# tsinghua-fib-lab/DRL-urban-planning

Measured on NVIDIA H100. Metric: ppo_update_graph_samples_per_sec, higher is better.
Workload: dtype f32

## Files before the change

drl_urban_planning_b200/csrc/optim_kernels.cuh:

```cuda
#pragma once
#include <cuda_runtime.h>
#include <stdint.h>

#include "../../include/upb200.h"
#include "layout.h"

namespace upb {

template <class L>
__device__ __forceinline__ bool chain_owns(int col) {
  return (col >= L::chain0_begin && col < L::chain0_end) || (col >= L::chain1_begin && col < L::chain1_end);
}

template <class L>
__device__ __forceinline__ bool write_grad_col(float* grad, int col, float v) {
  bool param = false;
  if (col < L::num_params && !chain_owns<L>(col)) { grad[col] = v; param = true; }
  else if (col >= L::num_params && col < L::stat_offset) grad[col] = 0.f;
  if (col >= L::stats && col < L::stats + UPB_STAT_COUNT)
    grad[L::stat_offset + (col - L::stats)] = stat_summed(col - L::stats) ? v : 0.f;
  return param;
}

constexpr int KL_STOP_SLOT = 13;
// ... 40 lines not shown
}

__device__ __forceinline__ double gclip_block_tree(double s, double* red) {
#pragma unroll
  for (int o = 16; o > 0; o >>= 1) s += __shfl_xor_sync(0xffffffffu, s, o);
  if ((threadIdx.x & 31) == 0) red[threadIdx.x >> 5] = s;
  __syncthreads();
  double r = 0.0;
  if (threadIdx.x == 0)
    for (int w = 0; w < GCLIP_BLOCK / 32; ++w) r += red[w];
  return r;
}

__device__ __forceinline__ float gclip_norm(const double* parts, int n) {
  double s = 0.0;
  for (int i = 0; i < n; ++i) s += parts[i];
  return (float)sqrt(s);
}

__device__ __forceinline__ float gclip_coef(float norm, float max_norm) {
  const float c = __fmul_rn(__frcp_rn(__fadd_rn(norm, 1e-6f)), max_norm);
  return c > 1.f ? 1.f : c;
}

template <class L>
__device__ __forceinline__ float column_sum4(const float* __restrict__ gpart, int nparts, int col) {
  float s0 = 0.f, s1 = 0.f, s2 = 0.f, s3 = 0.f;
  int c = 0;
  for (; c + 4 <= nparts; c += 4) {
    s0 += gpart[(size_t)(c + 0) * L::row + col];
    s1 += gpart[(size_t)(c + 1) * L::row + col];
    s2 += gpart[(size_t)(c + 2) * L::row + col];
    s3 += gpart[(size_t)(c + 3) * L::row + col];
  }
  for (; c < nparts; ++c) s0 += gpart[(size_t)c * L::row + col];
  return (s0 + s1) + (s2 + s3);
}

__device__ __forceinline__ void attention_chain(int t, const float* sG, const float* sWin, const float* sW,
                                                const float* sB, float* gW, int w_stride, float* gWin, float* gB,
                                                int b_stride, float* gBin) {
  const int r = t >> 4, c = t & 15;
  const int gC[3] = {0, 272, 528};
  const int gBo[3] = {256, -1, 784};
#pragma unroll
  for (int s = 0; s < 3; ++s) {
    const float* Win = sWin + s * 256;
    const float* gc = sG + gC[s];
    const float* W = sW + s * 256;
    float a = 0.f, b = 0.f;
#pragma unroll
    for (int rr = 0; rr < 16; ++rr) {
      a = fmaf(Win[rr * 16 + r], gc[rr * 16 + c], a);
      b = fmaf(gc[r * 16 + rr], W[c * 16 + rr], b);
    }
    if (gBo[s] >= 0) b = fmaf(sG[gBo[s] + r], sB[s * 16 + c], b);
    gW[s * w_stride + t] = a;
    gWin[s * 256 + t] = b;
    if (t < 16) {
      float gb = 0.f, gbin = 0.f;
      if (gBo[s] >= 0) {
        for (int rr = 0; rr < 16; ++rr) gb = fmaf(Win[rr * 16 + t], sG[gBo[s] + rr], gb);
        gbin = sG[gBo[s] + t];
      }
      gB[s * b_stride + t] = gb;
      gBin[s * 16 + t] = gbin;
    }
  }
}

constexpr int RF_THREADS = 256;
constexpr int RF_BLOCKS = (G_ROW + RF_THREADS - 1) / RF_THREADS;
static_assert(P_ATT_K_W - P_ATT_Q_W == P_ATT_V_W - P_ATT_K_W && P_ATT_K_B - P_ATT_Q_B == P_ATT_V_B - P_ATT_K_B,
              "q / k / v projections at a fixed stride");

__global__ void __launch_bounds__(RF_THREADS) k_reduce_finish(const float* __restrict__ gpart, int nparts,
                                                              float* __restrict__ gsum, const float* __restrict__ P,
                                                              float* __restrict__ grad, unsigned int* ticket,
                                                              const unsigned int* kl_stop) {
  __shared__ float sG[816];
  __shared__ float sWin[768];
  __shared__ float sW[768];
  __shared__ float sB[48];
  __shared__ bool is_last;
  const int t = threadIdx.x;
  const int idx = blockIdx.x * RF_THREADS + t;
  if (kl_stop && kl_stop_set(kl_stop)) {
    if (idx < UPB_GRAD_STRIDE) write_skip_elem(grad, UPB_STAT_OFFSET, idx);
    return;
  }
  if (idx < G_ROW) {
    const float v = column_sum4<SgnnRow>(gpart, nparts, idx);
    gsum[idx] = v;
    write_grad_col<SgnnRow>(grad, idx, v);
  }
  __threadfence();
  __syncthreads();
  if (t == 0) is_last = (atomicAdd(ticket, 1u) == gridDim.x - 1);
  __syncthreads();
  if (!is_last) return;
  __threadfence();
  if (t == 0) *ticket = 0u;
  for (int i = t; i < 816; i += RF_THREADS) sG[i] = __ldcg(gsum + G_QC + i);
  for (int i = t; i < 768; i += RF_THREADS) sWin[i] = P[P_MHA_IN_W + i];
  sW[t] = P[P_ATT_Q_W + t];
  sW[256 + t] = P[P_ATT_K_W + t];
  sW[512 + t] = P[P_ATT_V_W + t];
  if (t < 16) { sB[t] = P[P_ATT_Q_B + t]; sB[16 + t] = P[P_ATT_K_B + t]; sB[32 + t] = P[P_ATT_V_B + t]; }
  __syncthreads();
  attention_chain(t, sG, sWin, sW, sB, grad + P_ATT_Q_W, P_ATT_K_W - P_ATT_Q_W, grad + P_MHA_IN_W, grad + P_ATT_Q_B,
                  P_ATT_K_B - P_ATT_Q_B, grad + P_MHA_IN_B);
}

struct ApplyArgs {
  float* params;
  float* grad;
  float* m;
  float* v;
  const long long* steps_in;
  long long* steps_out;
  float lr, beta1, beta2, eps;
  float weight_decay;
  int clip_now;
  int num_params, encoder_end, policy_end, lu_begin, rd_begin, stat_offset;
  unsigned int* kl_stop;
  float kl_limit;
  float max_norm;
  int nslice;
  int chain0_begin, chain0_end, chain1_begin, chain1_end;
  int nonfinite_guard;
};

constexpr int AP_THREADS = 512;
constexpr int AP_PER_THREAD = 2;
constexpr int AP_BLOCKS = (NUM_PARAMS + AP_THREADS * AP_PER_THREAD - 1) / (AP_THREADS * AP_PER_THREAD);

__device__ __forceinline__ float block_sum_ap(float v, float* red) {
#pragma unroll
  for (int o = 16; o > 0; o >>= 1) v += __shfl_xor_sync(0xffffffffu, v, o);
  if ((threadIdx.x & 31) == 0) red[threadIdx.x >> 5] = v;
  __syncthreads();
  float s = 0.f;
  for (int w = 0; w < AP_THREADS / 32; ++w) s += red[w];
  __syncthreads();
  return s;
}

static_assert(AP_THREADS == GCLIP_BLOCK, "k_apply forms the chain partial with the chain CTA's tree");
constexpr int GCLIP_MAX_PARTS = 128;
__device__ __noinline__ float apply_gclip_norm(const ApplyArgs& a) {
  __shared__ double parts[GCLIP_MAX_PARTS];
  __shared__ double red[GCLIP_BLOCK / 32];
  __shared__ float norm;
  const int t = threadIdx.x, lane = t & 31;
  for (int sl = t >> 5; sl < a.nslice; sl += AP_THREADS / 32) {
    double x[4];
#pragma unroll
    for (int k = 0; k < 4; ++k) {
      const int col = sl * SLICE + lane + 32 * k;
      const bool real = col < a.num_params && !(col >= a.chain0_begin && col < a.chain0_end) &&
// ... 217 lines not shown
```

drl_urban_planning_b200/csrc/sgnn_kernel.cuh:

```cuda
#pragma once
#include <cuda_runtime.h>
#include <math_constants.h>
#include <stdint.h>

#include "blob.h"
#include "layout.h"
#include "optim_kernels.cuh"

namespace upb {

constexpr int NT = 512;
constexpr int NW = NT / 32;
constexpr int NS = 464;
constexpr int AS = 5632;
constexpr int KS = 160;
constexpr int CH = 96;
constexpr float MASK_FILL = -4294967296.0f;
constexpr float EPS_DEG = 1e-6f;

constexpr int S_WET = 0;
constexpr int S_BE = S_WET + 384;
constexpr int S_WPQ0 = S_BE + 16;
constexpr int S_B0 = S_WPQ0 + 512;
constexpr int S_WPQ1 = S_B0 + 16;
// ... 120 lines not shown
struct StepArgs {
  const uint8_t* blob;
  const int* ids;
  int count;
  const float* params;
  const float* actions;
  const float* adv;
  const float* ret;
  const float* fixed_lp;
  const float* exps;
  float inv_batch, inv_ind;
  float clip_lo, clip_hi;
  float c_value, c_entropy;
  int diagnostics;
  float* out_value;
  float* out_logp;
  float* out_entropy;
  int* out_greedy;
  const float* uniforms;
  int* out_sample;
  float* gpart;
  float* scratch;
  size_t scratch_stride;
  int n_cap, e_cap;
  int fuse_tail;
  float* params_rw;
  float* grad_out;
  float* adam_m;
  float* adam_v;
  const long long* steps_in;
  long long* steps_out;
  unsigned int* gridbar;
  unsigned int bar_target;
  float lr, beta1, beta2, adam_eps;
  float weight_decay;
  int world, rank;
  unsigned int seq;
  float* const* peers;
  long long* stamps;
  const int* logit_rows;
  float* lu_logits;
  float* rd_logits;
  unsigned int* kl_stop;
  float kl_limit;
  const float* old_values;
  float value_clip;
  float max_norm;
  float* out_cand_logp;
  const float* old_cand_logp;
  float kl_coef;
  int nonfinite_guard;
};

__device__ __forceinline__ float ex2_approx(float x) {
  float y;
  asm("ex2.approx.ftz.f32 %0, %1;" : "=f"(y) : "f"(x));
  return y;
}
__device__ __forceinline__ float rcp_approx(float x) {
  float y;
  asm("rcp.approx.ftz.f32 %0, %1;" : "=f"(y) : "f"(x));
  return y;
}
__device__ __forceinline__ float exp2a(float a) {
  const float t = fminf(fmaxf(a * 2.8853900817779268f, -115.41560327111707f), 115.41560327111707f);
  return ex2_approx(t);
}
__device__ __forceinline__ void cp_async16(void* smem_dst, const void* gsrc) {
  const unsigned d = (unsigned)__cvta_generic_to_shared(smem_dst);
  asm volatile("cp.async.cg.shared.global [%0], [%1], 16;" ::"r"(d), "l"(gsrc) : "memory");
}
__device__ __forceinline__ void cp_async_commit() { asm volatile("cp.async.commit_group;" ::: "memory"); }
__device__ __forceinline__ void cp_async_wait_all() { asm volatile("cp.async.wait_group 0;" ::: "memory"); }

__device__ __forceinline__ unsigned smem_u32(const void* p) { return (unsigned)__cvta_generic_to_shared(p); }
__device__ __forceinline__ void mbar_init(uint64_t* bar, unsigned count) {
  asm volatile("mbarrier.init.shared::cta.b64 [%0], %1;" ::"r"(smem_u32(bar)), "r"(count) : "memory");
}
__device__ __forceinline__ void fence_mbar_init() { asm volatile("fence.mbarrier_init.release.cluster;" ::: "memory"); }
__device__ __forceinline__ void fence_proxy_async() { asm volatile("fence.proxy.async;" ::: "memory"); }
__device__ __forceinline__ void mbar_expect_tx(uint64_t* bar, unsigned bytes) {
  asm volatile("mbarrier.arrive.expect_tx.shared::cta.b64 _, [%0], %1;" ::"r"(smem_u32(bar)), "r"(bytes) : "memory");
}
__device__ __forceinline__ void bulk_g2s(void* smem_dst, const void* gsrc, unsigned bytes, uint64_t* bar) {
  asm volatile("cp.async.bulk.shared::cluster.global.mbarrier::complete_tx::bytes [%0], [%1], %2, [%3];"
               ::"r"(smem_u32(smem_dst)), "l"(gsrc), "r"(bytes), "r"(smem_u32(bar)) : "memory");
}
__device__ __forceinline__ void mbar_wait(uint64_t* bar, unsigned parity) {
  asm volatile(
      "{\n\t.reg .pred p;\n\t"
      "WAIT_%=:\n\t"
      "mbarrier.try_wait.parity.shared::cta.b64 p, [%0], %1;\n\t"
      "@p bra DONE_%=;\n\t"
      "bra WAIT_%=;\n\t"
      "DONE_%=:\n\t}"
      ::"r"(smem_u32(bar)), "r"(parity) : "memory");
}

__device__ __forceinline__ float4 ld4(const float* p) { return *reinterpret_cast<const float4*>(p); }
__device__ __forceinline__ void st4(float* p, float4 v) { *reinterpret_cast<float4*>(p) = v; }
__device__ __forceinline__ float4 f4(float a) { return make_float4(a, a, a, a); }
__device__ __forceinline__ float4 operator+(float4 a, float4 b) { return make_float4(a.x + b.x, a.y + b.y, a.z + b.z, a.w + b.w); }
__device__ __forceinline__ float4 operator*(float4 a, float s) { return make_float4(a.x * s, a.y * s, a.z * s, a.w * s); }
__device__ __forceinline__ float4 operator*(float4 a, float4 b) { return make_float4(a.x * b.x, a.y * b.y, a.z * b.z, a.w * b.w); }
__device__ __forceinline__ float dot4(float4 a, float4 b) { return a.x * b.x + a.y * b.y + a.z * b.z + a.w * b.w; }
__device__ __forceinline__ float comp(const float4& v, int j) { return j == 0 ? v.x : j == 1 ? v.y : j == 2 ? v.z : v.w; }
// ... 1770 lines not shown
      } else if (sh.stop && col == L::stats + KL_STOP_SLOT) {
        a.grad_out[L::stat_offset + KL_STOP_SLOT] = 1.f;
        *a.kl_stop = 1u;
      }
    }
    __syncthreads();
  }
}

__device__ __forceinline__ void tail_write_steps(const StepArgs& a, const TailShared& sh) {
  const int tid = threadIdx.x;
  const bool live_lu = sh.bits & 1u, live_rd = sh.bits & 2u;
  if (sh.timeout == 0 && !sh.stop)
    a.steps_out[tid] = tid == 0 ? a.steps_in[0] + 1
                                : sh.steps[(tid - 1) * 2 + (tid == 1 ? 1 : (tid == 2 ? (live_lu ? 1 : 0) : (live_rd ? 1 : 0)))];
  else
    a.steps_out[tid] = a.steps_in[tid];
}

__device__ __forceinline__ void tail_count_timeout(const StepArgs& a, const TailShared& sh) {
  if (threadIdx.x == 0 && sh.timeout) atomicAdd(a.gridbar + 6, 1u);
}

template <class L>
__device__ __noinline__ void tail_kl_gate(const StepArgs& a, TailShared& sh, const float* pull, const unsigned* myflags,
                                          bool sys) {
  if ((int)threadIdx.x < a.world) tail_poll(a, sh, myflags, threadIdx.x, L::stats / SLICE, sys);
  __syncthreads();
  if (threadIdx.x == 0) {
    float s4 = ld_relaxed(pull + L::stats + 4, sys), s8 = ld_relaxed(pull + L::stats + 8, sys);
    for (int p = 1; p < a.world; ++p) {
      s4 += ld_relaxed(pull + (size_t)p * G_ROW + L::stats + 4, sys);
      s8 += ld_relaxed(pull + (size_t)p * G_ROW + L::stats + 8, sys);
    }
    sh.stop = sh.timeout == 0 && kl_exceeds(s8, s4, a.kl_limit);
  }
  __syncthreads();
}

template <bool STEPS>
__device__ __forceinline__ void tail_chain_grads(const StepArgs& a, TailShared& sh, const float* pull,
                                                 const unsigned* myflags, bool sys, float* chain) {
  float* sG = chain;
  float* sWin = sG + 816;
  float* sW3 = sWin + 768;
  float* sB = sW3 + 768;
  float* sOut = sB + 48;
  const int tid = threadIdx.x, world = a.world;
  {
    constexpr int NCH = CHAIN_S1 - CHAIN_S0 + 1;
    if (tid < world * NCH) tail_poll(a, sh, myflags, tid % world, CHAIN_S0 + tid / world, sys);
    __syncthreads();
  }
  if constexpr (STEPS) {
    if (tid < 4) tail_write_steps(a, sh);
  }
  {
    float v0[MAX_PEERS], v1[MAX_PEERS];
#pragma unroll
    for (int p = 0; p < MAX_PEERS; ++p) {
      v0[p] = 0.f; v1[p] = 0.f;
      if (p < world) {
        v0[p] = ld_relaxed(pull + (size_t)p * G_ROW + G_QC + tid, sys);
        if (tid + NT < 816) v1[p] = ld_relaxed(pull + (size_t)p * G_ROW + G_QC + tid + NT, sys);
      }
    }
    float s0 = v0[0], s1 = v1[0];
#pragma unroll
    for (int p = 1; p < MAX_PEERS; ++p) if (p < world) { s0 += v0[p]; s1 += v1[p]; }
    sG[tid] = s0;
    if (tid + NT < 816) sG[tid + NT] = s1;
  }
  __syncthreads();
  if (tid < 256) attention_chain(tid, sG, sWin, sW3, sB, sOut, 256, sOut + 768, sOut + 1536, 16, sOut + 1584);
  __syncthreads();
}

template <class L>
__device__ __forceinline__ void tail_gclip(const StepArgs& a, TailShared& sh, const float* pull,
                                           const unsigned* myflags, bool sys, int c, bool active, double* sq,
                                           float* chain) {
  constexpr bool CHAIN = L::chain0_end > L::chain0_begin;
  constexpr int NPARTS = L::nslice + (CHAIN ? 1 : 0);
  static_assert(NPARTS <= FLAG_STRIDE, "a flag word per partial");
  double* const sparts = sq + SLICE;
  float& snorm = *reinterpret_cast<float*>(sparts + FLAG_STRIDE);
  float& scoef = *(&snorm + 1);
  const int tid = threadIdx.x, world = a.world;
  const unsigned par = a.seq & 1u;
  float* const mine = a.peers[a.rank];
  double* const parts = reinterpret_cast<double*>(mine + XCHG_GCLIP) + (size_t)par * FLAG_STRIDE;
  unsigned* const pflags = reinterpret_cast<unsigned*>(mine + XCHG_GCLIP_FLAGS) + (size_t)par * FLAG_STRIDE;
  const bool stop = sh.stop;

  for (int sl = blockIdx.x; sl < L::nslice; sl += gridDim.x) {
    if (tid < world) tail_poll(a, sh, myflags, tid, sl, sys);
    __syncthreads();
    const int col = sl * SLICE + c;
    if (active) {
      double x = 0.0;
      if (L::row % SLICE == 0 || col < L::row) {
        const float s = rank_sum(pull, world, col, sys);
        if (write_grad_col<L>(a.grad_out, col, s)) x = (double)s * (double)s;
        else if (stop && col == L::stats + KL_STOP_SLOT) {
          a.grad_out[L::stat_offset + KL_STOP_SLOT] = 1.f;
          *a.kl_stop = 1u;
// ... 58 lines not shown
  __syncthreads();

  const float norm = snorm, coef = scoef;
  const bool bad = a.nonfinite_guard && !isfinite(norm);
  const bool dead = sh.timeout != 0 || bad;
  const bool live_lu = sh.bits & 1u, live_rd = sh.bits & 2u;
  if (active) {
    for (int sl = blockIdx.x; sl < L::nslice; sl += gridDim.x) {
      const int col = sl * SLICE + c;
      if (col < L::num_params && !chain_owns<L>(col)) {
        int seg = 0;
        bool live = true;
        if (col >= L::lu_begin && col < L::rd_begin) { seg = 1; live = live_lu; }
        else if (col >= L::rd_begin && col < L::policy_end) { seg = 2; live = live_rd; }
        if (live && !dead)
          adam_elem(a, col, __fmul_rn(a.grad_out[col], coef), a.adam_m[col], a.adam_v[col], a.params_rw[col],
                    sh.adam[(seg * 2 + 1) * 2], sh.adam[(seg * 2 + 1) * 2 + 1]);
      } else if (col == L::stats + GCLIP_NORM_SLOT && !dead && a.max_norm > 0.f) {
        a.grad_out[L::stat_offset + GCLIP_NORM_SLOT] = norm;
      } else if (col == L::stats + NONFINITE_SLOT && bad && sh.timeout == 0) {
        a.grad_out[L::stat_offset + NONFINITE_SLOT] = 1.f;
      }
    }
  }
  if constexpr (CHAIN) {
    if (chain != nullptr && !dead) {
      const float* sOut = chain + 2400;
#pragma unroll
      for (int j = 0; j < 4; ++j) {
        const int i = tid + j * GCLIP_BLOCK;
        if (i < CHAIN_ELEMS) {
          const int dst = chain_dst(i);
          adam_elem(a, dst, __fmul_rn(sOut[i], coef), a.adam_m[dst], a.adam_v[dst], a.params_rw[dst], sh.adam[2],
                    sh.adam[3]);
        }
      }
    }
  }
}

template <class L>
__device__ __noinline__ void skip_step(const StepArgs& a) {
  if (!a.fuse_tail) return;
  const int tid = threadIdx.x;
  for (int i = blockIdx.x * blockDim.x + tid; i < L::stat_offset + UPB_STAT_COUNT; i += gridDim.x * blockDim.x)
    write_skip_elem(a.grad_out, L::stat_offset, i);
  if (blockIdx.x == 0) {
    if (tid < 4) a.steps_out[tid] = a.steps_in[tid];
    if (tid == 4) a.gridbar[2 + ((a.seq & 1u) ^ 1u)] = 0u;
  }
  grid_arrive(a.gridbar);
}

template <bool GCLIP>
__device__ __forceinline__ void fused_tail(const StepArgs& a, float* smem, unsigned stage_bits) {
  const int tid = threadIdx.x;
  const int nparts = gridDim.x;
  const int world = a.world, me = a.rank;
  const bool sys = world > 1;
  const unsigned par = a.seq & 1u;
  const bool chain_cta = blockIdx.x == gridDim.x - 1;
  __shared__ TailShared sh;
#define UPB_TSTAMP(ID) do { if (a.stamps != nullptr && blockIdx.x == 0 && threadIdx.x == 0) a.stamps[ID] = clock64(); } while (0)
  UPB_TSTAMP(40);
  float* const mine = a.peers[me];
  const float* const pull = mine + (size_t)par * MAX_PEERS * G_ROW;
  const unsigned* const myflags = reinterpret_cast<const unsigned*>(mine + XCHG_FLAGS) + (size_t)par * MAX_PEERS * FLAG_STRIDE;
  tail_prologue(a, sh, stage_bits);
  const int col0 = blockIdx.x * SLICE + (tid >> 2), part = tid & 3;
  float pm = 0.f, pv = 0.f, pp = 0.f;
  if (!GCLIP && part == 0 && col0 < NUM_PARAMS && !chain_owns<SgnnRow>(col0)) {
    pm = a.adam_m[col0]; pv = a.adam_v[col0]; pp = a.params_rw[col0];
  }
  float* sG = smem;
  float* sWin = sG + 816;
  float* sW3 = sWin + 768;
  float* sB = sW3 + 768;
  float* sOut = sB + 48;
  const int pW[3] = {P_ATT_Q_W, P_ATT_K_W, P_ATT_V_W};
  const int pB[3] = {P_ATT_Q_B, P_ATT_K_B, P_ATT_V_B};
  float cm[4], cv[4], cp[4];
  int cdst[4];
  if (chain_cta) {
    const float* P = a.params_rw;
    for (int i = tid; i < 768; i += NT) sWin[i] = P[P_MHA_IN_W + i];
    if (tid < 256) { sW3[tid] = P[P_ATT_Q_W + tid]; sW3[256 + tid] = P[P_ATT_K_W + tid]; sW3[512 + tid] = P[P_ATT_V_W + tid]; }
    if (tid < 16) { sB[tid] = P[P_ATT_Q_B + tid]; sB[16 + tid] = P[P_ATT_K_B + tid]; sB[32 + tid] = P[P_ATT_V_B + tid]; }
#pragma unroll
    for (int j = 0; j < 4; ++j) {
      const int i = tid + j * NT;
      int dst = 0;
      if (i < 768) dst = pW[i >> 8] + (i & 255);
      else if (i < 1536) dst = P_MHA_IN_W + (i - 768);
      else if (i < 1584) dst = pB[(i - 1536) >> 4] + ((i - 1536) & 15);
      else if (i < 1632) dst = P_MHA_IN_B + (i - 1584);
      cdst[j] = dst;
      if (!GCLIP && i < 1632) { cm[j] = a.adam_m[dst]; cv[j] = a.adam_v[dst]; cp[j] = P[dst]; }
    }
  }
  const unsigned flagword = tail_barrier(a);
  UPB_TSTAMP(41);

  float* sPart = smem + 4096;
  for (int sl = blockIdx.x; sl < NSLICE; sl += gridDim.x) {
    const int lane = tid & 31, warp = tid >> 5, cg = warp & 3, rg = warp >> 2;
    const float* src = a.gpart + sl * SLICE + cg * 32 + lane;
    float s = 0.f;
    for (int r0 = rg; r0 < nparts; r0 += 160) {
      float t[40];
#pragma unroll
      for (int j = 0; j < 40; ++j) t[j] = r0 + 4 * j < nparts ? __ldcg(src + (size_t)(r0 + 4 * j) * G_ROW) : 0.f;
#pragma unroll
      for (int w = 1; w < 40; w <<= 1)
#pragma unroll
        for (int j = 0; j + w < 40; j += 2 * w) t[j] += t[j + w];
      s += t[0];
    }
    __syncthreads();
    sPart[rg * SLICE + cg * 32 + lane] = s;
    __syncthreads();
    if (tid < SLICE) {
      const float v = (sPart[tid] + sPart[SLICE + tid]) + (sPart[2 * SLICE + tid] + sPart[3 * SLICE + tid]);
      const int col = sl * SLICE + tid;
      for (int r = 0; r < world; ++r) st_relaxed(sh.push[r] + col, v, sys);
    }
  }
  tail_release<SgnnRow>(a, flagword, NT, sys);
  if (a.kl_stop) tail_kl_gate<SgnnRow>(a, sh, pull, myflags, sys);
  UPB_TSTAMP(42);
  if constexpr (GCLIP) {
    tail_gclip<SgnnRow>(a, sh, pull, myflags, sys, tid >> 2, part == 0, reinterpret_cast<double*>(sPart + 4 * SLICE),
                        chain_cta ? smem : nullptr);
    if (chain_cta && tid < 4) tail_write_steps(a, sh);
    tail_count_timeout(a, sh);
    return;
  }

  tail_reduce_adam<SgnnRow>(a, sh, pull, myflags, sys, tid >> 2, part == 0, col0, pm, pv, pp);
  UPB_TSTAMP(43);
  if (!chain_cta) {
    tail_count_timeout(a, sh);
    return;
  }

  tail_chain_grads<true>(a, sh, pull, myflags, sys, sG);
  const bool dead = sh.timeout != 0 || sh.stop;
#pragma unroll
  for (int j = 0; j < 4; ++j) {
    const int i = tid + j * NT;
    if (i < 1632) {
      const float g = sOut[i];
      a.grad_out[cdst[j]] = g;
      if (!dead) adam_elem(a, cdst[j], g, cm[j], cv[j], cp[j], sh.adam[2], sh.adam[3]);
    }
  }
  tail_count_timeout(a, sh);
  UPB_TSTAMP(44);
}

template <bool TRAIN, bool GCLIP>
__device__ __forceinline__ void sgnn_step(const StepArgs& a) {
  extern __shared__ __align__(16) float smem[];
  __shared__ __align__(8) uint64_t s_mbar[4];
  if constexpr (TRAIN) {
    if (a.kl_stop && kl_stop_set(a.kl_stop)) {
      skip_step<SgnnRow>(a);
      return;
    }
  }
  const long long t_cta0 = a.stamps ? clock64() : 0;
  if (a.stamps && threadIdx.x == 0 && blockIdx.x == 0) {
    unsigned long long gt;
    asm volatile("mov.u64 %0, %%globaltimer;" : "=l"(gt));
    a.stamps[30] = t_cta0; a.stamps[32] = (long long)gt;
  }
  if (threadIdx.x == 0) {
    mbar_init(s_mbar + 0, 1); mbar_init(s_mbar + 1, 1); mbar_init(s_mbar + 2, 1); mbar_init(s_mbar + 3, 1);
    fence_mbar_init();
  }
  unsigned nstaged = 0;
  load_weights(a.params, smem);
  float* gp = nullptr;
  if constexpr (TRAIN) {
    gp = a.gpart + (size_t)blockIdx.x * G_ROW;
    for (int i = threadIdx.x; i < G_ROW / 4; i += NT) reinterpret_cast<float4*>(gp)[i] = f4(0.f);
  }
  __syncthreads();
  if (a.stamps && threadIdx.x == 0 && blockIdx.x < 160) a.stamps[64 + 160 + blockIdx.x] = clock64() - t_cta0;
  const BlobHeader& hd = *reinterpret_cast<const BlobHeader*>(a.blob);
  const GraphDesc* descs = reinterpret_cast<const GraphDesc*>(a.blob + hd.off_desc);
  float* scr = a.scratch + (size_t)blockIdx.x * a.scratch_stride;
  unsigned stage_bits = 0;
  for (int item = blockIdx.x; item < a.count; item += gridDim.x) {
    const int gid = a.ids ? a.ids[item] : item;
    const GraphDesc d = descs[gid];
    stage_bits |= 1u << (d.stage & 1);
    if (d.n > a.n_cap || d.e > a.e_cap || d.n < 1) {
      if (threadIdx.x == 0) {
        if constexpr (TRAIN) gacc(gp, G_STATS + 7, 1.f);
        if (a.out_value) a.out_value[gid] = CUDART_NAN_F;
        if (a.out_logp) a.out_logp[gid] = CUDART_NAN_F;
        if (a.out_entropy) a.out_entropy[gid] = CUDART_NAN_F;
      }
      if constexpr (!TRAIN) { write_skipped_logit_row<NT>(a, gid, d.stage); write_skipped_cand_logp<NT>(a, d); }
      continue;
    }
    if (item + (int)gridDim.x < a.count) prefetch_next_graph<TRAIN>(a, item + gridDim.x);
    const bool big = d.n > NS || 2 * d.e > AS || d.k > KS || d.ord_rounds > ORD_ROUNDS;
    if (big) graph_body<TRAIN, true>(a, hd, d, gid, smem, gp, scr, item == (int)(blockIdx.x + gridDim.x), s_mbar, 0u);
    else { graph_body<TRAIN, false>(a, hd, d, gid, smem, gp, scr, item == (int)(blockIdx.x + gridDim.x), s_mbar, nstaged & 1u); ++nstaged; }
    __syncthreads();
  }
  if (a.stamps && threadIdx.x == 0 && blockIdx.x < 160) a.stamps[64 + blockIdx.x] = clock64() - t_cta0;
  if (a.stamps && threadIdx.x == 0 && blockIdx.x == 0) {
    unsigned long long gt;
    asm volatile("mov.u64 %0, %%globaltimer;" : "=l"(gt));
    a.stamps[31] = clock64(); a.stamps[33] = (long long)gt;
  }
  if constexpr (TRAIN) {
    if (a.fuse_tail) fused_tail<GCLIP>(a, smem, stage_bits);
  }
}

template <bool TRAIN>
__global__ void __launch_bounds__(NT, 1) k_sgnn(const __grid_constant__ StepArgs a) {
  sgnn_step<TRAIN, false>(a);
}
__global__ void __launch_bounds__(NT, 1) k_sgnn_gclip(const __grid_constant__ StepArgs a) {
  sgnn_step<true, true>(a);
}

}
```

drl_urban_planning_b200/csrc/upb200.cu:

```cuda
#include <cuda_runtime.h>

#include <cmath>
#include <cstdio>
#include <cstring>
#include <new>
#include <string>
#include <utility>
#include <vector>

#include "../../include/upb200.h"
#include "blob.h"
#include "errors.h"
#include "layout.h"
#include "optim_kernels.cuh"
#include "sgnn_kernel.cuh"
#include "mlp_kernel.cuh"

using namespace upb;

struct Model {
  void (*train)(StepArgs);
  void (*infer)(StepArgs);
  int threads;
  size_t smem;
// ... 73 lines not shown
  } while (0)

struct Slot {
  const char* name;
  int offset, rows, cols;
};
const Slot kSlots[] = {
    {"num_w0", P_NUM_W0, 64, 52},      {"num_b0", P_NUM_B0, 64, 0},     {"num_w1", P_NUM_W1, 16, 64},
    {"num_b1", P_NUM_B1, 16, 0},       {"enc_w", P_ENC_W, 16, 23},      {"enc_b", P_ENC_B, 16, 0},
    {"gcn0_w", P_GCN0_W, 16, 32},      {"gcn0_b", P_GCN0_B, 16, 0},     {"gcn1_w", P_GCN1_W, 16, 32},
    {"gcn1_b", P_GCN1_B, 16, 0},       {"mha_in_w", P_MHA_IN_W, 48, 16}, {"mha_in_b", P_MHA_IN_B, 48, 0},
    {"mha_out_w", P_MHA_OUT_W, 16, 16}, {"mha_out_b", P_MHA_OUT_B, 16, 0}, {"att_q_w", P_ATT_Q_W, 16, 16},
    {"att_q_b", P_ATT_Q_B, 16, 0},     {"att_k_w", P_ATT_K_W, 16, 16},  {"att_k_b", P_ATT_K_B, 16, 0},
    {"att_v_w", P_ATT_V_W, 16, 16},    {"att_v_b", P_ATT_V_B, 16, 0},   {"lu_w0", P_LU_W0, 32, 64},
    {"lu_b0", P_LU_B0, 32, 0},         {"lu_w1", P_LU_W1, 1, 32},       {"road_w0", P_RD_W0, 32, 16},
    {"road_b0", P_RD_B0, 32, 0},       {"road_w1", P_RD_W1, 1, 32},     {"val_w0", P_VAL_W0, 32, 67},
    {"val_b0", P_VAL_B0, 32, 0},       {"val_w1", P_VAL_W1, 32, 32},    {"val_b1", P_VAL_B1, 32, 0},
    {"val_w2", P_VAL_W2, 1, 32},       {"val_b2", P_VAL_B2, 1, 0},
};
constexpr int kNumSlots = sizeof(kSlots) / sizeof(kSlots[0]);

using ModelOf = Model upb_ctx::*;

int check_ctx(const upb_ctx* ctx, const char* who) {
  if (!ctx) return set_error(UPB_ERR_ARG, std::string(who) + ": null context");
  return UPB_OK;
}
int bad_argument(const char* who) { return set_error(UPB_ERR_ARG, std::string(who) + ": bad argument"); }

bool prof_begin(upb_ctx* ctx, cudaStream_t s) {
  if (!ctx->profiling) return false;
  if (ctx->prof_used == ctx->prof_events.size()) {
    cudaEvent_t a, b;
    if (cudaEventCreate(&a) != cudaSuccess || cudaEventCreate(&b) != cudaSuccess) return false;
    ctx->prof_events.emplace_back(a, b);
  }
  cudaEventRecord(ctx->prof_events[ctx->prof_used].first, s);
  return true;
}
void prof_end(upb_ctx* ctx, cudaStream_t s, bool on) {
  if (!on) return;
  cudaEventRecord(ctx->prof_events[ctx->prof_used].second, s);
  ctx->prof_used += 1;
}

bool clip_now(const upb_ctx* ctx, const Model& m) {
  return ctx->cfg.clip_mode == UPB_CLIP_ALWAYS || (ctx->cfg.clip_mode == UPB_CLIP_REFERENCE && m.clip_armed);
}

int model_init(upb_ctx* ctx, Model& m) {
  if (m.gpart) return UPB_OK;
  m.scratch_stride = (m.scratch_floats(ctx->cfg.n_cap, ctx->cfg.e_cap) + 63) & ~size_t(63);
  UPB_CUDA(cudaMalloc(&m.gpart, sizeof(float) * (size_t)ctx->grid * m.row));
  UPB_CUDA(cudaMalloc(&m.scratch, sizeof(float) * (size_t)ctx->grid * m.scratch_stride));
  UPB_CUDA(cudaMalloc(&m.adam_m, sizeof(float) * m.num_params));
  UPB_CUDA(cudaMalloc(&m.adam_v, sizeof(float) * m.num_params));
  UPB_CUDA(cudaMalloc(&m.steps, sizeof(long long) * 8));
  UPB_CUDA(cudaMalloc(&m.kl_stop, sizeof(unsigned int)));
  UPB_CUDA(cudaMemset(m.kl_stop, 0, sizeof(unsigned int)));
  UPB_CUDA(cudaMemset(m.adam_m, 0, sizeof(float) * m.num_params));
  UPB_CUDA(cudaMemset(m.adam_v, 0, sizeof(float) * m.num_params));
  UPB_CUDA(cudaMemset(m.steps, 0, sizeof(long long) * 8));
  UPB_CUDA(cudaMemset(m.scratch, 0, sizeof(float) * (size_t)ctx->grid * m.scratch_stride));
  UPB_CUDA(cudaFuncSetAttribute(m.train, cudaFuncAttributeMaxDynamicSharedMemorySize, (int)m.smem));
  UPB_CUDA(cudaFuncSetAttribute(m.infer, cudaFuncAttributeMaxDynamicSharedMemorySize, (int)m.smem));
  UPB_CUDA(cudaFuncSetAttribute(m.train_gclip, cudaFuncAttributeMaxDynamicSharedMemorySize, (int)m.smem));
  UPB_CUDA(cudaDeviceSynchronize());
  return UPB_OK;
}

void model_free(Model& m) {
  cudaFree(m.gpart);
  cudaFree(m.scratch);
  cudaFree(m.adam_m);
  cudaFree(m.adam_v);
  cudaFree(m.steps);
  cudaFree(m.kl_stop);
}

void reduce_sgnn(const upb_ctx* ctx, int nparts, const float* params, float* grad, const unsigned int* kl_stop,
                 cudaStream_t s) {
  k_reduce_finish<<<RF_BLOCKS, RF_THREADS, 0, s>>>(ctx->sgnn.gpart, nparts, ctx->gsum, params, grad, ctx->ticket,
                                                   kl_stop);
}
void reduce_mlp(const upb_ctx* ctx, int nparts, const float*, float* grad, const unsigned int* kl_stop,
                cudaStream_t s) {
  k_mlp_reduce<<<(MG_ROW + 255) / 256, 256, 0, s>>>(ctx->mlp.gpart, nparts, grad, kl_stop);
}

unsigned int* kl_stop_word(const upb_ctx* ctx, const Model& m) { return ctx->kl_limit > 0.f ? m.kl_stop : nullptr; }

StepArgs step_args(const upb_ctx* ctx, const Model& m, const void* blob, const int32_t* ids, int count,
                   const float* params, const float* actions) {
  StepArgs a;
  memset(&a, 0, sizeof(a));
  a.blob = (const uint8_t*)blob;
  a.ids = ids;
  a.count = count;
  a.params = params;
  a.actions = actions;
  a.clip_lo = ctx->clip_lo;
  a.clip_hi = ctx->clip_hi;
  a.c_value = ctx->cfg.value_pred_coef;
  a.c_entropy = ctx->cfg.entropy_coef;
  a.diagnostics = ctx->diagnostics ? 1 : 0;
  a.gpart = m.gpart;
// ... 739 lines not shown
```

drl_urban_planning_b200/engine.py:

```python
from __future__ import annotations

import ctypes as C
import math
from typing import Optional, Tuple

import numpy as np
import torch

from . import _lib
from .packing import PackedGraphs


def _ptr(t: Optional[torch.Tensor]) -> Optional[int]:
    return None if t is None else t.data_ptr()


def _f32(t: torch.Tensor, device) -> torch.Tensor:
    if t.device != device or t.dtype != torch.float32 or not t.is_contiguous():
        t = t.to(device=device, dtype=torch.float32).contiguous()
    return t


def _cpulist(text: str):
    out = []
# ... 391 lines not shown
                      ) -> None:
        m = np.ascontiguousarray(m, np.float32)
        v = np.ascontiguousarray(v, np.float32)
        steps = np.ascontiguousarray(steps, np.int64)
        assert m.size == self.num_params and v.size == self.num_params
        _lib.check(getattr(_lib.lib(), self._p + "set_opt_state")(self._ctx, m.ctypes.data, v.ctypes.data,
                                                                 steps.ctypes.data), self._p + "set_opt_state")
        if rearm_first_step_clip:
            _lib.check(getattr(_lib.lib(), self._p + "rearm_clip")(self._ctx), self._p + "rearm_clip")

    def profile(self, enable: bool) -> None:
        _lib.check(_lib.lib().upb_profile_enable(self._ctx, int(enable)), "upb_profile_enable")

    def profile_read(self):
        ms, n = C.c_double(), C.c_int()
        _lib.check(_lib.lib().upb_profile_read(self._ctx, C.byref(ms), C.byref(n)), "upb_profile_read")
        return float(ms.value), int(n.value)

    @property
    def grid(self) -> int:
        return int(_lib.lib().upb_grid_size(self._ctx))

    @staticmethod
    def graph_cost(info: np.ndarray) -> np.ndarray:
        i = np.asarray(info, dtype=np.int64)
        return 17 * i[:, 1] + 80 * i[:, 0] + 134 * i[:, 2] + 41500

    def balance_ids(self, ids: np.ndarray, cost: np.ndarray) -> np.ndarray:
        import heapq
        ids = np.asarray(ids)
        g = self.grid
        if len(ids) <= g:
            return ids[np.argsort(-np.asarray(cost)[ids], kind="stable")]
        c = np.asarray(cost, dtype=np.float64)[ids]
        order = np.argsort(-c, kind="stable")
        m = len(ids)
        if m <= 2 * g and c[order[0]] < c[order[g - 1]] + c[order[-1]]:
            srt = ids[order]
            npair = m - g
            return np.concatenate([srt[g - npair:g], srt[:g - npair], srt[m - 1:g - 1:-1] if npair else srt[:0]])
        bins = [[] for _ in range(g)]
        heap = [(0.0, b) for b in range(g)]
        for k in order:
            load, b = heapq.heappop(heap)
            bins[b].append(int(ids[k]))
            heapq.heappush(heap, (load + float(c[k]), b))
        bins.sort(key=lambda x: -len(x))
        out = []
        for r in range(len(bins[0])):
            row = [b[r] for b in bins if len(b) > r]
            out.extend(row)
        return np.asarray(out, dtype=ids.dtype)

    def set_stamp_buffer(self, buf: Optional[torch.Tensor]) -> None:
        _lib.check(_lib.lib().upb_set_stamp_buffer(self._ctx, _ptr(buf)), "upb_set_stamp_buffer")

    @property
    def launches(self) -> int:
        return int(_lib.lib().upb_launch_count(self._ctx))
```

include/upb200.h:

```cpp
#ifndef UPB200_H_
#define UPB200_H_

#include <stddef.h>
#include <stdint.h>

#ifdef __cplusplus
extern "C" {
#endif

#define UPB_ABI_VERSION 1

#define UPB_NODE_DIM 23
#define UPB_NODE_STRIDE 24
#define UPB_NUMERICAL_DIM 52
#define UPB_GCN_DIM 16
#define UPB_NUM_GCN_LAYERS 2
#define UPB_NUM_PARAMS 13729
#define UPB_GRAD_STRIDE 13760
#define UPB_STAT_OFFSET 13732
#define UPB_STAT_COUNT 28

#define UPB_MLP_NUM_PARAMS 10257
#define UPB_MLP_STAT_OFFSET 10260
#define UPB_MLP_GRAD_STRIDE 10288
// ... 118 lines not shown
int upb_set_target_kl(upb_ctx* ctx, float target_kl);
int upb_reset_kl_stop(upb_ctx* ctx, void* stream);
int upb_mlp_reset_kl_stop(upb_ctx* ctx, void* stream);
int upb_set_clip_range(upb_ctx* ctx, float lo, float hi);

int upb_set_value_clip(upb_ctx* ctx, float value_clip);
int upb_ppo_grad_vclip(upb_ctx* ctx, const void* blob_dev, const int32_t* ids, int count, const float* params,
                       const float* actions, const float* advantages, const float* returns,
                       const float* fixed_log_probs, const float* exps, const float* old_values, float inv_batch,
                       float inv_ind, float* grad_out, void* stream);
int upb_ppo_step_vclip(upb_ctx* ctx, const void* blob_dev, const int32_t* ids, int count, float* params,
                       const float* actions, const float* advantages, const float* returns,
                       const float* fixed_log_probs, const float* exps, const float* old_values, float inv_batch,
                       float inv_ind, float* grad_out, void* stream);
int upb_mlp_ppo_grad_vclip(upb_ctx* ctx, const void* blob_dev, const int32_t* ids, int count, const float* params,
                           const float* actions, const float* advantages, const float* returns,
                           const float* fixed_log_probs, const float* exps, const float* old_values, float inv_batch,
                           float inv_ind, float* grad_out, void* stream);
int upb_mlp_ppo_step_vclip(upb_ctx* ctx, const void* blob_dev, const int32_t* ids, int count, float* params,
                           const float* actions, const float* advantages, const float* returns,
                           const float* fixed_log_probs, const float* exps, const float* old_values, float inv_batch,
                           float inv_ind, float* grad_out, void* stream);
typedef struct {
  const float* old_values;
  const float* old_cand_log_probs;
} upb_step_refs;
int upb_ppo_grad_refs(upb_ctx* ctx, const void* blob_dev, const int32_t* ids, int count, const float* params,
                      const float* actions, const float* advantages, const float* returns,
                      const float* fixed_log_probs, const float* exps, const upb_step_refs* refs, float inv_batch,
                      float inv_ind, float* grad_out, void* stream);
int upb_ppo_step_refs(upb_ctx* ctx, const void* blob_dev, const int32_t* ids, int count, float* params,
                      const float* actions, const float* advantages, const float* returns,
                      const float* fixed_log_probs, const float* exps, const upb_step_refs* refs, float inv_batch,
                      float inv_ind, float* grad_out, void* stream);
int upb_mlp_ppo_grad_refs(upb_ctx* ctx, const void* blob_dev, const int32_t* ids, int count, const float* params,
                          const float* actions, const float* advantages, const float* returns,
                          const float* fixed_log_probs, const float* exps, const upb_step_refs* refs,
                          float inv_batch, float inv_ind, float* grad_out, void* stream);
int upb_mlp_ppo_step_refs(upb_ctx* ctx, const void* blob_dev, const int32_t* ids, int count, float* params,
                          const float* actions, const float* advantages, const float* returns,
                          const float* fixed_log_probs, const float* exps, const upb_step_refs* refs,
                          float inv_batch, float inv_ind, float* grad_out, void* stream);
int upb_set_kl_penalty(upb_ctx* ctx, float beta);
int upb_set_max_grad_norm(upb_ctx* ctx, float max_norm);
int upb_set_nonfinite_guard(upb_ctx* ctx, int enable);
int upb_normalize_advantages(upb_ctx* ctx, const float* adv_in, const float* exps, const int32_t* order, int T_used,
                             int B, float* adv_out, void* stream);

int upb_profile_enable(upb_ctx* ctx, int enable);
int upb_profile_read(upb_ctx* ctx, double* total_ms, int* launches);

int upb_grid_size(const upb_ctx* ctx);

int upb_set_stamp_buffer(upb_ctx* ctx, void* stamps_dev);

int64_t upb_launch_count(const upb_ctx* ctx);

#ifdef __cplusplus
}
#endif
#endif
```

Baseline: 1.740 million.

## Zero gradient partials in tail, transpose attention weights, add timeline stamps

```diff
diff --git a/drl_urban_planning_b200/csrc/optim_kernels.cuh b/drl_urban_planning_b200/csrc/optim_kernels.cuh
--- a/drl_urban_planning_b200/csrc/optim_kernels.cuh
+++ b/drl_urban_planning_b200/csrc/optim_kernels.cuh
@@ -116,7 +116,7 @@
 #pragma unroll
     for (int rr = 0; rr < 16; ++rr) {
       a = fmaf(Win[rr * 16 + r], gc[rr * 16 + c], a);
-      b = fmaf(gc[r * 16 + rr], W[c * 16 + rr], b);
+      b = fmaf(gc[r * 16 + rr], W[rr * 16 + c], b);
     }
     if (gBo[s] >= 0) b = fmaf(sG[gBo[s] + r], sB[s * 16 + c], b);
     gW[s * w_stride + t] = a;
@@ -138,7 +138,7 @@
 static_assert(P_ATT_K_W - P_ATT_Q_W == P_ATT_V_W - P_ATT_K_W && P_ATT_K_B - P_ATT_Q_B == P_ATT_V_B - P_ATT_K_B,
               "q / k / v projections at a fixed stride");
 
-__global__ void __launch_bounds__(RF_THREADS) k_reduce_finish(const float* __restrict__ gpart, int nparts,
+__global__ void __launch_bounds__(RF_THREADS) k_reduce_finish(float* __restrict__ gpart, int nparts,
                                                               float* __restrict__ gsum, const float* __restrict__ P,
                                                               float* __restrict__ grad, unsigned int* ticket,
                                                               const unsigned int* kl_stop) {
@@ -155,6 +155,7 @@
   }
   if (idx < G_ROW) {
     const float v = column_sum4<SgnnRow>(gpart, nparts, idx);
+    for (int c = 0; c < nparts; ++c) gpart[(size_t)c * G_ROW + idx] = 0.f;
     gsum[idx] = v;
     write_grad_col<SgnnRow>(grad, idx, v);
   }
@@ -167,9 +168,10 @@
   if (t == 0) *ticket = 0u;
   for (int i = t; i < 816; i += RF_THREADS) sG[i] = __ldcg(gsum + G_QC + i);
   for (int i = t; i < 768; i += RF_THREADS) sWin[i] = P[P_MHA_IN_W + i];
-  sW[t] = P[P_ATT_Q_W + t];
-  sW[256 + t] = P[P_ATT_K_W + t];
-  sW[512 + t] = P[P_ATT_V_W + t];
+  const int tr = (t & 15) * 16 + (t >> 4);
+  sW[tr] = P[P_ATT_Q_W + t];
+  sW[256 + tr] = P[P_ATT_K_W + t];
+  sW[512 + tr] = P[P_ATT_V_W + t];
   if (t < 16) { sB[t] = P[P_ATT_Q_B + t]; sB[16 + t] = P[P_ATT_K_B + t]; sB[32 + t] = P[P_ATT_V_B + t]; }
   __syncthreads();
   attention_chain(t, sG, sWin, sW, sB, grad + P_ATT_Q_W, P_ATT_K_W - P_ATT_Q_W, grad + P_MHA_IN_W, grad + P_ATT_Q_B,
diff --git a/drl_urban_planning_b200/csrc/sgnn_kernel.cuh b/drl_urban_planning_b200/csrc/sgnn_kernel.cuh
--- a/drl_urban_planning_b200/csrc/sgnn_kernel.cuh
+++ b/drl_urban_planning_b200/csrc/sgnn_kernel.cuh
@@ -196,6 +196,33 @@
   int nonfinite_guard;
 };
 
+constexpr int TL_BASE = 384, TL_CTAS = 160;
+enum TlPoint {
+  TL_ENTRY,
+  TL_PROLOGUE,
+  TL_GRAPH,
+  TL_LOOP_END = TL_GRAPH + 4,
+  TL_BARRIER,
+  TL_PUSH,
+  TL_ADAM,
+  TL_CHAIN_WAIT,
+  TL_CHAIN,
+  TL_EXIT,
+  TL_POINTS
+};
+constexpr int TL_GRAPHS = TL_LOOP_END - TL_GRAPH;
+static_assert(TL_BASE + 2 * TL_POINTS * TL_CTAS == UPB_STAMP_WORDS, "the stamp buffer's size (upb200.h)");
+__device__ __forceinline__ void tl_stamp(long long* s, int p) {
+  unsigned long long gt;
+  asm volatile("mov.u64 %0, %%globaltimer;" : "=l"(gt));
+  s[TL_BASE + p * TL_CTAS + blockIdx.x] = (long long)gt;
+  s[TL_BASE + (TL_POINTS + p) * TL_CTAS + blockIdx.x] = clock64();
+}
+#define UPB_TL(P)                                                                                    \
+  do {                                                                                               \
+    if (a.stamps != nullptr && threadIdx.x == 0 && blockIdx.x < TL_CTAS) tl_stamp(a.stamps, (P)); \
+  } while (0)
+
 __device__ __forceinline__ float ex2_approx(float x) {
   float y;
   asm("ex2.approx.ftz.f32 %0, %1;" : "=f"(y) : "f"(x));
@@ -2072,6 +2099,7 @@
     if (tid < world * NCH) tail_poll(a, sh, myflags, tid % world, CHAIN_S0 + tid / world, sys);
     __syncthreads();
   }
+  UPB_TL(TL_CHAIN_WAIT);
   if constexpr (STEPS) {
     if (tid < 4) tail_write_steps(a, sh);
   }
@@ -2236,6 +2264,12 @@
   grid_arrive(a.gridbar);
 }
 
+__device__ __forceinline__ void zero_owned_slices(const StepArgs& a) {
+  for (int sl = blockIdx.x; sl < NSLICE; sl += gridDim.x)
+    for (int i = threadIdx.x; i < (int)gridDim.x * (SLICE / 4); i += blockDim.x)
+      reinterpret_cast<float4*>(a.gpart + (size_t)(i / (SLICE / 4)) * G_ROW + sl * SLICE)[i % (SLICE / 4)] = f4(0.f);
+}
+
 template <bool GCLIP>
 __device__ __forceinline__ void fused_tail(const StepArgs& a, float* smem, unsigned stage_bits) {
   const int tid = threadIdx.x;
@@ -2268,7 +2302,10 @@
   if (chain_cta) {
     const float* P = a.params_rw;
     for (int i = tid; i < 768; i += NT) sWin[i] = P[P_MHA_IN_W + i];
-    if (tid < 256) { sW3[tid] = P[P_ATT_Q_W + tid]; sW3[256 + tid] = P[P_ATT_K_W + tid]; sW3[512 + tid] = P[P_ATT_V_W + tid]; }
+    if (tid < 256) {
+      const int tr = (tid & 15) * 16 + (tid >> 4);
+      sW3[tr] = P[P_ATT_Q_W + tid]; sW3[256 + tr] = P[P_ATT_K_W + tid]; sW3[512 + tr] = P[P_ATT_V_W + tid];
+    }
     if (tid < 16) { sB[tid] = P[P_ATT_Q_B + tid]; sB[16 + tid] = P[P_ATT_K_B + tid]; sB[32 + tid] = P[P_ATT_V_B + tid]; }
 #pragma unroll
     for (int j = 0; j < 4; ++j) {
@@ -2284,6 +2321,7 @@
   }
   const unsigned flagword = tail_barrier(a);
   UPB_TSTAMP(41);
+  UPB_TL(TL_BARRIER);
 
   float* sPart = smem + 4096;
   for (int sl = blockIdx.x; sl < NSLICE; sl += gridDim.x) {
@@ -2312,18 +2350,22 @@
   tail_release<SgnnRow>(a, flagword, NT, sys);
   if (a.kl_stop) tail_kl_gate<SgnnRow>(a, sh, pull, myflags, sys);
   UPB_TSTAMP(42);
+  UPB_TL(TL_PUSH);
   if constexpr (GCLIP) {
     tail_gclip<SgnnRow>(a, sh, pull, myflags, sys, tid >> 2, part == 0, reinterpret_cast<double*>(sPart + 4 * SLICE),
                         chain_cta ? smem : nullptr);
     if (chain_cta && tid < 4) tail_write_steps(a, sh);
     tail_count_timeout(a, sh);
+    zero_owned_slices(a);
     return;
   }
 
   tail_reduce_adam<SgnnRow>(a, sh, pull, myflags, sys, tid >> 2, part == 0, col0, pm, pv, pp);
   UPB_TSTAMP(43);
+  UPB_TL(TL_ADAM);
   if (!chain_cta) {
     tail_count_timeout(a, sh);
+    zero_owned_slices(a);
     return;
   }
 
@@ -2340,6 +2382,8 @@
   }
   tail_count_timeout(a, sh);
   UPB_TSTAMP(44);
+  UPB_TL(TL_CHAIN);
+  zero_owned_slices(a);
 }
 
 template <bool TRAIN, bool GCLIP>
@@ -2352,6 +2396,7 @@
       return;
     }
   }
+  UPB_TL(TL_ENTRY);
   const long long t_cta0 = a.stamps ? clock64() : 0;
   if (a.stamps && threadIdx.x == 0 && blockIdx.x == 0) {
     unsigned long long gt;
@@ -2365,12 +2410,10 @@
   unsigned nstaged = 0;
   load_weights(a.params, smem);
   float* gp = nullptr;
-  if constexpr (TRAIN) {
-    gp = a.gpart + (size_t)blockIdx.x * G_ROW;
-    for (int i = threadIdx.x; i < G_ROW / 4; i += NT) reinterpret_cast<float4*>(gp)[i] = f4(0.f);
-  }
+  if constexpr (TRAIN) gp = a.gpart + (size_t)blockIdx.x * G_ROW;
   __syncthreads();
   if (a.stamps && threadIdx.x == 0 && blockIdx.x < 160) a.stamps[64 + 160 + blockIdx.x] = clock64() - t_cta0;
+  UPB_TL(TL_PROLOGUE);
   const BlobHeader& hd = *reinterpret_cast<const BlobHeader*>(a.blob);
   const GraphDesc* descs = reinterpret_cast<const GraphDesc*>(a.blob + hd.off_desc);
   float* scr = a.scratch + (size_t)blockIdx.x * a.scratch_stride;
@@ -2394,8 +2437,11 @@
     if (big) graph_body<TRAIN, true>(a, hd, d, gid, smem, gp, scr, item == (int)(blockIdx.x + gridDim.x), s_mbar, 0u);
     else { graph_body<TRAIN, false>(a, hd, d, gid, smem, gp, scr, item == (int)(blockIdx.x + gridDim.x), s_mbar, nstaged & 1u); ++nstaged; }
     __syncthreads();
+    const int round = (item - (int)blockIdx.x) / (int)gridDim.x;
+    if (round < TL_GRAPHS) UPB_TL(TL_GRAPH + round);
   }
   if (a.stamps && threadIdx.x == 0 && blockIdx.x < 160) a.stamps[64 + blockIdx.x] = clock64() - t_cta0;
+  UPB_TL(TL_LOOP_END);
   if (a.stamps && threadIdx.x == 0 && blockIdx.x == 0) {
     unsigned long long gt;
     asm volatile("mov.u64 %0, %%globaltimer;" : "=l"(gt));
@@ -2404,6 +2450,7 @@
   if constexpr (TRAIN) {
     if (a.fuse_tail) fused_tail<GCLIP>(a, smem, stage_bits);
   }
+  UPB_TL(TL_EXIT);
 }
 
 template <bool TRAIN>
diff --git a/drl_urban_planning_b200/csrc/upb200.cu b/drl_urban_planning_b200/csrc/upb200.cu
--- a/drl_urban_planning_b200/csrc/upb200.cu
+++ b/drl_urban_planning_b200/csrc/upb200.cu
@@ -149,6 +149,7 @@
   if (m.gpart) return UPB_OK;
   m.scratch_stride = (m.scratch_floats(ctx->cfg.n_cap, ctx->cfg.e_cap) + 63) & ~size_t(63);
   UPB_CUDA(cudaMalloc(&m.gpart, sizeof(float) * (size_t)ctx->grid * m.row));
+  UPB_CUDA(cudaMemset(m.gpart, 0, sizeof(float) * (size_t)ctx->grid * m.row));
   UPB_CUDA(cudaMalloc(&m.scratch, sizeof(float) * (size_t)ctx->grid * m.scratch_stride));
   UPB_CUDA(cudaMalloc(&m.adam_m, sizeof(float) * m.num_params));
   UPB_CUDA(cudaMalloc(&m.adam_v, sizeof(float) * m.num_params));
diff --git a/drl_urban_planning_b200/engine.py b/drl_urban_planning_b200/engine.py
--- a/drl_urban_planning_b200/engine.py
+++ b/drl_urban_planning_b200/engine.py
@@ -467,7 +467,11 @@
             out.extend(row)
         return np.asarray(out, dtype=ids.dtype)
 
+    STAMP_WORDS = 4544
+
     def set_stamp_buffer(self, buf: Optional[torch.Tensor]) -> None:
+        if buf is not None and (buf.dtype != torch.int64 or not buf.is_cuda or buf.numel() < self.STAMP_WORDS):
+            raise ValueError(f"the stamp buffer must be a CUDA int64 tensor of at least {self.STAMP_WORDS} words")
         _lib.check(_lib.lib().upb_set_stamp_buffer(self._ctx, _ptr(buf)), "upb_set_stamp_buffer")
 
     @property
diff --git a/include/upb200.h b/include/upb200.h
--- a/include/upb200.h
+++ b/include/upb200.h
@@ -194,6 +194,7 @@
 
 int upb_grid_size(const upb_ctx* ctx);
 
+#define UPB_STAMP_WORDS 4544
 int upb_set_stamp_buffer(upb_ctx* ctx, void* stamps_dev);
 
 int64_t upb_launch_count(const upb_ctx* ctx);
```

Measured after the change: 1.753 million, median of 6. About the same (+0.8%).
